# jesselasse/MARL-DMFB

Hardware: AMD Instinct MI355X
Metric: env-steps/sec (whole node), 10x10 DMFB 4-droplet fov9 (higher is better)
Workload: dtype int8 env state/obs + f64 rewards; fp32 Q-net; 1 GPU; DMFB 10x10, drop_num=4, fov=9, 4096 parallel envs per GPU (BASELINE configs[1]); parallelism=dp1: chips sharded per rank, one flat RCCL all-reduce per learn

## Files before the change

marl_dmfb_amd/csrc/gru_ops.hip:

```cpp
#include <hip/hip_runtime.h>

#include <cstdint>
#include <cstdio>
#include <cstdlib>

#include "../../include/crnn_ops.h"

#define HIP_ABI_TAG "crnn_ops"
#define HIP_ABI_ERR CRNN_ERR_HIP
#include "hip_abi.h"

namespace {

constexpr int kBlock = 512;
constexpr int H = 128;
constexpr int RW = 8;
constexpr int KQ = 32;

__device__ __forceinline__ float sigmoidf_(float x) { return 1.0f / (1.0f + __expf(-x)); }

struct SeqOff {
    int32_t packed;
    int32_t off[GRU_SEQ_MAX_STEPS + 1];
};

typedef float f32x2 __attribute__((ext_vector_type(2)));
typedef float f32x4 __attribute__((ext_vector_type(4)));

__global__ __launch_bounds__(kBlock) void k_gru_seq_fwd(const float *__restrict__ igates, const float *__restrict__ h0,
                                                        const float *__restrict__ w_hh, const float *__restrict__ b_ih,
                                                        const float *__restrict__ b_hh, int T, long R,
                                                        float *__restrict__ hs, float *__restrict__ gates, const SeqOff so) {
    __shared__ __attribute__((aligned(16))) float s_h[RW / 2][H][2];
    __shared__ __attribute__((aligned(16))) float s_part[4][RW][3][H];
    const int tid = threadIdx.x, q = tid / H, u = tid - q * H;
    const long row0 = (long)blockIdx.x * RW;
    const int rv = (int)min((long)RW, R - row0);
    f32x4 w[3][KQ / 4];
#pragma unroll
    for (int g = 0; g < 3; ++g)
#pragma unroll
        for (int k = 0; k < KQ / 4; ++k) w[g][k] = *(const f32x4 *)(w_hh + (size_t)(g * H + u) * H + q * KQ + 4 * k);
    const float bir = b_ih[u] + b_hh[u], biz = b_ih[H + u] + b_hh[H + u], bin = b_ih[2 * H + u], bhn = b_hh[2 * H + u];
    for (int i = tid; i < RW * H; i += kBlock) {
        const int rr = i / H, c = i - rr * H;
        s_h[rr >> 1][c][rr & 1] = rr < rv ? h0[(row0 + rr) * H + c] : 0.0f;
    }
    __syncthreads();
    const int ra = 2 * q;
    for (int t = 0; t < T; ++t) {
        const long rt = so.packed ? (long)(so.off[t + 1] - so.off[t]) : R;
        if (row0 >= rt) break;
        const int rvt = (int)min((long)rv, rt - row0);
        const size_t base = so.packed ? (size_t)so.off[t] : (size_t)t * R;
        float ig[2][3];
#pragma unroll
        for (int s = 0; s < 2; ++s) {
            const int rr = ra + s;
#pragma unroll
            for (int g = 0; g < 3; ++g) ig[s][g] = rr < rvt ? igates[(base + row0 + rr) * 3 * H + g * H + u] : 0.0f;
        }
#pragma unroll
        for (int rp = 0; rp < RW / 2; ++rp) {
            const f32x4 *ph = (const f32x4 *)(&s_h[rp][q * KQ][0]);
            f32x2 acc[3] = {{0.0f, 0.0f}, {0.0f, 0.0f}, {0.0f, 0.0f}};
#pragma unroll
            for (int j = 0; j < KQ / 4; ++j) {
                const f32x4 v0 = ph[2 * j], v1 = ph[2 * j + 1];
#pragma unroll
// ... 59 lines not shown
    const int ra = 2 * q;
    float gh[2] = {0.0f, 0.0f};
    float bs_r = 0.0f, bs_z = 0.0f, bs_n = 0.0f, bs_hn = 0.0f;
    int t_last = -1;
    for (int t = 0; t < T; ++t)
        if (row0 < (so.packed ? (long)(so.off[t + 1] - so.off[t]) : R)) t_last = t;
    struct In { float g, rg, zg, ng, hn, hp; };
    In cur[2], nx[2];
    auto fetch = [&](int t, In (&in)[2]) __attribute__((always_inline)) {
        const long rt = so.packed ? (long)(so.off[t + 1] - so.off[t]) : R;
        const int rvt = (int)min((long)rv, rt - row0);
        const size_t base = so.packed ? (size_t)so.off[t] : (size_t)t * R;
        const size_t base_prev = so.packed ? (size_t)so.off[t > 0 ? t - 1 : 0] : (size_t)(t > 0 ? t - 1 : 0) * R;
#pragma unroll
        for (int s = 0; s < 2; ++s) {
            const int rr = ra + s;
            const bool on = rr < rvt;
            const size_t o = base + row0 + (on ? rr : 0);
            in[s].g = on ? grad_hs[o * H + u] : 0.0f;
            in[s].rg = on ? gates[o * 4 * H + u] : 0.0f;
            in[s].zg = on ? gates[o * 4 * H + H + u] : 0.0f;
            in[s].ng = on ? gates[o * 4 * H + 2 * H + u] : 0.0f;
            in[s].hn = on ? gates[o * 4 * H + 3 * H + u] : 0.0f;
            in[s].hp = !on ? 0.0f : t > 0 ? hs[(base_prev + row0 + rr) * H + u] : h0[(row0 + rr) * H + u];
        }
    };
    if (t_last >= 0) fetch(t_last, cur);
    for (int t = t_last; t >= 0; --t) {
        const long rt = so.packed ? (long)(so.off[t + 1] - so.off[t]) : R;
        const int rvt = (int)min((long)rv, rt - row0);
        const size_t base = so.packed ? (size_t)so.off[t] : (size_t)t * R;
        float direct[2];
#pragma unroll
        for (int s = 0; s < 2; ++s) {
            const int rr = ra + s;
            float dpr = 0.0f, dpz = 0.0f, dpn = 0.0f, dhn = 0.0f;
            direct[s] = 0.0f;
            if (rr < rvt) {
                const size_t o = base + row0 + rr;
                const float g = cur[s].g + gh[s];
                const float rg = cur[s].rg, zg = cur[s].zg, ng = cur[s].ng, hn = cur[s].hn;
                const float hp = cur[s].hp;
                if (h_prev_out) h_prev_out[o * H + u] = hp;
                const float dn = g * (1.0f - zg), dz = g * (hp - ng);
                direct[s] = g * zg;
                dpn = dn * (1.0f - ng * ng);
                dhn = dpn * rg;
// ... 136 lines not shown

}

extern "C" {

static int make_seq_off(const int32_t *step_rows, int T, int64_t R, SeqOff &so) {
    so.packed = step_rows ? 1 : 0;
    if (!step_rows) return CRNN_OK;
    if (T > GRU_SEQ_MAX_STEPS) return CRNN_ERR_UNSUPPORTED;
    long off = 0, prev = R;
    for (int t = 0; t < T; ++t) {
        if (step_rows[t] < 0 || step_rows[t] > prev) return CRNN_ERR_BAD_ARG;
        so.off[t] = (int32_t)off;
        off += step_rows[t];
        prev = step_rows[t];
        if (off > 0x7fffffffL) return CRNN_ERR_BAD_ARG;
    }
    so.off[T] = (int32_t)off;
    return CRNN_OK;
}

static int seq_forward(const float *d_igates, const float *d_h0, const float *d_w_hh, const float *d_b_ih, const float *d_b_hh,
                       int T, int64_t R, int hidden, const int32_t *step_rows, float *d_hs, float *d_gates, void *stream) {
    if (!d_igates || !d_h0 || !d_w_hh || !d_b_ih || !d_b_hh || !d_hs || T < 0 || R < 0) return CRNN_ERR_BAD_ARG;
    if (hidden != H) return CRNN_ERR_UNSUPPORTED;
    if (T == 0 || R == 0) return CRNN_OK;
    SeqOff so;
    const int rc = make_seq_off(step_rows, T, R, so);
    if (rc != CRNN_OK) return rc;
    LAUNCH(k_gru_seq_fwd, dim3((unsigned)((R + RW - 1) / RW)), dim3(kBlock), 0, (hipStream_t)stream, d_igates, d_h0, d_w_hh,
           d_b_ih, d_b_hh, T, (long)R, d_hs, d_gates, so);
    return CRNN_OK;
}

int gru_seq_forward(const float *d_igates, const float *d_h0, const float *d_w_hh, const float *d_b_ih, const float *d_b_hh,
                    int T, int64_t R, int hidden, float *d_hs, float *d_gates, void *stream) {
    return seq_forward(d_igates, d_h0, d_w_hh, d_b_ih, d_b_hh, T, R, hidden, nullptr, d_hs, d_gates, stream);
}

int gru_seq_forward_packed(const float *d_igates, const float *d_h0, const float *d_w_hh, const float *d_b_ih, const float *d_b_hh,
                           int T, int64_t R, int hidden, const int32_t *step_rows, float *d_hs, float *d_gates, void *stream) {
    if (!step_rows) return CRNN_ERR_BAD_ARG;
    return seq_forward(d_igates, d_h0, d_w_hh, d_b_ih, d_b_hh, T, R, hidden, step_rows, d_hs, d_gates, stream);
}

int gru_seq_forward_packed_pair(const float *d_igates_a, const float *d_h0_a, const float *d_w_hh_a, const float *d_b_ih_a,
                                const float *d_b_hh_a, float *d_hs_a, float *d_gates_a, const float *d_igates_b, const float *d_h0_b,
                                const float *d_w_hh_b, const float *d_b_ih_b, const float *d_b_hh_b, float *d_hs_b, float *d_gates_b,
                                int T, int64_t R, int hidden, const int32_t *step_rows, void *stream) {
    if (!d_igates_a || !d_w_hh_a || !d_b_ih_a || !d_b_hh_a || !d_hs_a || T < 0 || R < 0 || !step_rows) return CRNN_ERR_BAD_ARG;
    const bool two = d_igates_b != nullptr;
    if (two && (!d_w_hh_b || !d_b_ih_b || !d_b_hh_b || !d_hs_b)) return CRNN_ERR_BAD_ARG;
    if ((((size_t)d_w_hh_a | (size_t)d_w_hh_b) & 15) != 0) return CRNN_ERR_BAD_ARG;
    if (hidden != H) return CRNN_ERR_UNSUPPORTED;
    if (T == 0 || R == 0) return CRNN_OK;
    SeqOff so;
    const int rc = make_seq_off(step_rows, T, R, so);
    if (rc != CRNN_OK) return rc;
    const long per_net = (R + kMW - 1) / kMW;
    if (per_net * 2 > 0x7fffffffL) return CRNN_ERR_BAD_ARG;
    const GruNetIO a{d_igates_a, d_h0_a, d_w_hh_a, d_b_ih_a, d_b_hh_a, d_hs_a, d_gates_a};
    const GruNetIO b{d_igates_b, d_h0_b, d_w_hh_b, d_b_ih_b, d_b_hh_b, d_hs_b, d_gates_b};
    LAUNCH(k_gru_seq_fwd_mfma, dim3((unsigned)(per_net * (two ? 2 : 1))), dim3(kBlock), 0, (hipStream_t)stream, a, two ? b : a,
           (int)per_net, T, (long)R, so);
    return CRNN_OK;
}

static int seq_backward(const float *d_grad_hs, const float *d_gates, const float *d_hs, const float *d_h0, const float *d_w_hh,
                        int T, int64_t R, int hidden, const int32_t *step_rows, float *d_d_igates, float *d_d_hgates, float *d_d_h0,
                        float *d_bias_part, void *stream, float *d_h_prev = nullptr) {
    if (!d_grad_hs || !d_gates || !d_hs || !d_h0 || !d_w_hh || !d_d_igates || !d_d_hgates || T < 0 || R < 0) return CRNN_ERR_BAD_ARG;
    if (hidden != H) return CRNN_ERR_UNSUPPORTED;
    if (T == 0 || R == 0) return CRNN_OK;
    SeqOff so;
    const int rc = make_seq_off(step_rows, T, R, so);
    if (rc != CRNN_OK) return rc;
    LAUNCH(k_gru_seq_bwd, dim3((unsigned)((R + RW - 1) / RW)), dim3(kBlock), 0, (hipStream_t)stream, d_grad_hs, d_gates, d_hs,
           d_h0, d_w_hh, T, (long)R, d_d_igates, d_d_hgates, d_d_h0, d_bias_part, so, d_h_prev);
    return CRNN_OK;
}

int gru_seq_backward(const float *d_grad_hs, const float *d_gates, const float *d_hs, const float *d_h0, const float *d_w_hh,
                     int T, int64_t R, int hidden, float *d_d_igates, float *d_d_hgates, float *d_d_h0, float *d_bias_part,
                     void *stream) {
    return seq_backward(d_grad_hs, d_gates, d_hs, d_h0, d_w_hh, T, R, hidden, nullptr, d_d_igates, d_d_hgates, d_d_h0, d_bias_part, stream);
}

int gru_seq_backward_packed(const float *d_grad_hs, const float *d_gates, const float *d_hs, const float *d_h0, const float *d_w_hh,
                            int T, int64_t R, int hidden, const int32_t *step_rows, float *d_d_igates, float *d_d_hgates,
                            float *d_d_h0, float *d_bias_part, float *d_h_prev, void *stream) {
    if (!step_rows) return CRNN_ERR_BAD_ARG;
    return seq_backward(d_grad_hs, d_gates, d_hs, d_h0, d_w_hh, T, R, hidden, step_rows, d_d_igates, d_d_hgates, d_d_h0, d_bias_part, stream,
                        d_h_prev);
}
// ... 7 lines not shown
```

marl_dmfb_amd/csrc/vdn_ops.hip:

```cpp
#include <hip/hip_runtime.h>

#include <cstdint>

#include "../../include/vdn_ops.h"
#include "../../include/vdn_tail.h"
#include "../../include/vdn_double.h"

#define HIP_ABI_TAG "vdn_ops"
#define HIP_ABI_ERR VDN_ERR_HIP
#include "hip_abi.h"

namespace {

__device__ unsigned g_td_ticket = 0;
__device__ __forceinline__ void td_block_sums(float sq, float mk, float *part, float *__restrict__ sums) {
    __shared__ float s_w[2][4];
    __shared__ int s_last;
    for (int o = 32; o > 0; o >>= 1) { sq += __shfl_xor(sq, o); mk += __shfl_xor(mk, o); }
    if ((threadIdx.x & 63) == 0) { s_w[0][threadIdx.x >> 6] = sq; s_w[1][threadIdx.x >> 6] = mk; }
    __syncthreads();
    if (threadIdx.x < 2) part[2 * blockIdx.x + threadIdx.x] = (s_w[threadIdx.x][0] + s_w[threadIdx.x][1]) + (s_w[threadIdx.x][2] + s_w[threadIdx.x][3]);
    if (!last_workgroup_arrives(&g_td_ticket, gridDim.x, &s_last)) return;
    if (threadIdx.x < 128) {
        const int which = threadIdx.x >> 6;
// ... 129 lines not shown
    }
    const int i = (int)(row % n);
    const UnitOf s = ix.unit(row / n);
    const float d = -((2.0f * mtd[s.row]) * maskf[s.row]) * g[0];
    const int a_taken = (int)u[s.ep * n + i];
    const bool bad_a = (unsigned)a_taken >= (unsigned)A;
    for (int a = 0; a < A; ++a) gq[row * A + a] = (bad_a || a == a_taken) ? d : 0.0f;
}

template <typename V>
__global__ __launch_bounds__(256) void k_gather_units(const V *__restrict__ src, int unit_v, const int32_t *__restrict__ units, int U, int shift,
                                                      int zero_below, V *__restrict__ dst) {
    const long idx = (long)blockIdx.x * blockDim.x + threadIdx.x;
    if (idx >= (long)U * unit_v) return;
    const int j = (int)(idx / unit_v), k = (int)(idx - (long)j * unit_v);
    dst[idx] = j < zero_below ? (V)0 : src[((size_t)units[j] + shift) * unit_v + k];
}

struct GatherBatch {
    const void *src[VDN_GATHER_MAX];
    void *dst[VDN_GATHER_MAX];
    long total[VDN_GATHER_MAX], total_pad[VDN_GATHER_MAX];
    int unit_v[VDN_GATHER_MAX], shift[VDN_GATHER_MAX], zero_below[VDN_GATHER_MAX], dw[VDN_GATHER_MAX];
};
template <typename V>
__device__ __forceinline__ void gather_word(const void *src, int unit_v, const int32_t *__restrict__ units, int shift, int zero_below,
                                            void *dst, long total, long idx) {
    V v = (V)0;
    if (idx < total) {
        const int j = (int)(idx / unit_v), k = (int)(idx - (long)j * unit_v);
        if (j >= zero_below) v = ((const V *)src)[((size_t)units[j] + shift) * unit_v + k];
    }
    ((V *)dst)[idx] = v;
}
__global__ __launch_bounds__(256) void k_gather_units_batch(GatherBatch gb, const int32_t *__restrict__ units) {
    const int d = blockIdx.y;
    const long idx = (long)blockIdx.x * blockDim.x + threadIdx.x;
    if (idx >= gb.total_pad[d]) return;
    if (gb.dw[d]) gather_word<uint32_t>(gb.src[d], gb.unit_v[d], units, gb.shift[d], gb.zero_below[d], gb.dst[d], gb.total[d], idx);
    else gather_word<uint8_t>(gb.src[d], gb.unit_v[d], units, gb.shift[d], gb.zero_below[d], gb.dst[d], gb.total[d], idx);
}

}

#include "vdn_lambda_kernels.h"
#include "vdn_double_kernels.h"

namespace {

struct TensorList {
    float *p[VDN_MAX_TENSORS];
    float *g[VDN_MAX_TENSORS];
    float *m[VDN_MAX_TENSORS];
    float *v[VDN_MAX_TENSORS];
    long off[VDN_MAX_TENSORS + 1];
    int n;
};

__device__ __forceinline__ void locate(const TensorList &tl, long i, int &k) {
    while (i >= tl.off[k + 1]) ++k;
}

__global__ __launch_bounds__(256) void k_sqnorm_partials(TensorList tl, float *__restrict__ partials, const float *__restrict__ grad_div) {
    __shared__ float s_w[4];
    const long total = tl.off[tl.n];
    const long per = (total + gridDim.x - 1) / gridDim.x;
    const long lo = (long)blockIdx.x * per, hi = min(total, lo + per);
    float acc = 0.0f;
    int k = 0;
    for (long i = lo + threadIdx.x; i < hi; i += 256) {
        locate(tl, i, k);
        float g = tl.g[k][i - tl.off[k]];
        if (grad_div) g = g / grad_div[0];
        acc = fmaf(g, g, acc);
    }
    for (int o = 32; o > 0; o >>= 1) acc += __shfl_xor(acc, o);
    if ((threadIdx.x & 63) == 0) s_w[threadIdx.x >> 6] = acc;
    __syncthreads();
    if (threadIdx.x == 0) partials[blockIdx.x] = (s_w[0] + s_w[1]) + (s_w[2] + s_w[3]);
}

__global__ __launch_bounds__(256) void k_clip_adam(TensorList tl, const float *__restrict__ partials, int n_partials, float max_norm,
                                                   float step_size, float omb1, float beta2, float omb2, float eps, float bc2_sqrt,
                                                   float *__restrict__ total_norm, const float *__restrict__ grad_div) {
    __shared__ float s_coef;
    if (threadIdx.x < 64) {
        float t = 0.0f;
        for (int b = threadIdx.x; b < n_partials; b += 64) t += partials[b];
        for (int o = 32; o > 0; o >>= 1) t += __shfl_xor(t, o);
        if (threadIdx.x == 0) {
            const float norm = sqrtf(t);
            s_coef = norm != norm ? norm : fminf(max_norm / (norm + 1e-6f), 1.0f);
            if (blockIdx.x == 0) total_norm[0] = norm;
        }
    }
    __syncthreads();
    const float coef = s_coef;
    const long total = tl.off[tl.n];
    const long per = (total + gridDim.x - 1) / gridDim.x;
    const long lo = (long)blockIdx.x * per, hi = min(total, lo + per);
    int k = 0;
    for (long i = lo + threadIdx.x; i < hi; i += 256) {
        locate(tl, i, k);
        const long j = i - tl.off[k];
        float g = tl.g[k][j];
        if (grad_div) g = g / grad_div[0];
        g = g * coef;
        if (grad_div || coef != 1.0f) tl.g[k][j] = g;
        float m = tl.m[k][j], v = tl.v[k][j];
        m = m + omb1 * (g - m);
        v = beta2 * v + omb2 * g * g;
        tl.m[k][j] = m;
        tl.v[k][j] = v;
        const float denom = sqrtf(v) / bc2_sqrt + eps;
        tl.p[k][j] -= step_size * (m / denom);
    }
}

bool td_forward_args_ok(const TdIn &in, const TdOut &out) {
    return !(out.sums && !out.part) && in.qe && in.qt && in.u && in.r && in.avail && in.term && in.padded && out.mtd && out.maskf && in.n >= 1 &&
           in.A >= 1 && in.A <= 127;
}
bool td_backward_args_ok(const float *mtd, const float *mask, const int8_t *u, const float *g, const float *gq, int n, int A) {
    return mtd && mask && u && g && gq && n >= 1 && A >= 1 && A <= 127;
}
bool padded_shape_ok(int B, int T, int Tl) { return B >= 0 && T >= 1 && Tl >= T; }

int td_no_rows(const TdOut &out, void *stream) {
    if (out.sums) HIP_TRY(hipMemsetAsync(out.sums, 0, 2 * sizeof(float), (hipStream_t)stream));
    return VDN_OK;
}

bool lambda_padded_args_ok(const TdIn &in, const TdOut &out, int B, int T, int Tl, float lam) {
    return td_forward_args_ok(in, out) && padded_shape_ok(B, T, Tl) && T <= VDN_LAMBDA_MAX_T && lam >= 0.0f && lam <= 1.0f &&
           (int64_t)B * T <= 0x7fffffffL;
}
bool lambda_packed_args_ok(const TdIn &in, const TdOut &out, const int32_t *units, int n_units, float lam, int n_steps) {
    return td_forward_args_ok(in, out) && units && n_units >= 0 && lam >= 0.0f && lam <= 1.0f && n_steps >= 0 && n_steps <= VDN_LAMBDA_MAX_T;
// ... 224 lines not shown
    return VDN_OK;
}

int vdn_gather_units_batch(int32_t n_gathers, const void *const *d_src, const int32_t *unit_bytes, const int32_t *unit_shift,
                           const int32_t *zero_below, void *const *d_dst, const int64_t *dst_bytes, const int32_t *d_units,
                           int32_t n_units, void *stream) {
    if (n_gathers < 1 || n_gathers > VDN_GATHER_MAX || !d_src || !unit_bytes || !unit_shift || !zero_below || !d_dst || !dst_bytes ||
        !d_units || n_units < 0)
        return VDN_ERR_BAD_ARG;
    GatherBatch gb{};
    long most = 0;
    for (int i = 0; i < n_gathers; ++i) {
        if (!d_src[i] || !d_dst[i] || unit_bytes[i] < 1 || zero_below[i] < 0 || dst_bytes[i] < (int64_t)n_units * unit_bytes[i])
            return VDN_ERR_BAD_ARG;
        const bool dw = unit_bytes[i] % 4 == 0 && dst_bytes[i] % 4 == 0 && ((size_t)d_src[i] | (size_t)d_dst[i]) % 4 == 0;
        gb.src[i] = d_src[i];
        gb.dst[i] = d_dst[i];
        gb.dw[i] = dw ? 1 : 0;
        gb.unit_v[i] = dw ? unit_bytes[i] / 4 : unit_bytes[i];
        gb.total[i] = (long)n_units * gb.unit_v[i];
        gb.total_pad[i] = (long)(dw ? dst_bytes[i] / 4 : dst_bytes[i]);
        gb.shift[i] = unit_shift[i];
        gb.zero_below[i] = zero_below[i];
        most = gb.total_pad[i] > most ? gb.total_pad[i] : most;
    }
    if (most == 0) return VDN_OK;
    if ((most + 255) / 256 > 0x7fffffffL) return VDN_ERR_BAD_ARG;
    LAUNCH(k_gather_units_batch, dim3((unsigned)((most + 255) / 256), (unsigned)n_gathers), dim3(256), 0, (hipStream_t)stream, gb, d_units);
    return VDN_OK;
}

int vdn_last_hip_error(void) { return g_last_hip; }

}
```

marl_dmfb_amd/network/base_net.py:

```python

import torch
import torch.nn as nn
import torch.nn.functional as f


_CONV_PLAN = {5: [(True, 1)], 7: [(True, 1), (False, 1)], 9: [(True, 1), (False, 1)], 11: [(True, 1), (False, 1)],
              13: [(True, 1), (False, 1)], 19: [(True, 2), (False, 1), (False, 1)]}


class _ConvGemm(torch.autograd.Function):

    @staticmethod
    def forward(ctx, cols, weight2d, bias):
        ctx.save_for_backward(cols, weight2d)
        return torch.addmm(bias, cols, weight2d.t())

    @staticmethod
    def backward(ctx, g):
        cols, w = ctx.saved_tensors
        g = g.contiguous()
        gcols = g @ w if ctx.needs_input_grad[0] else None
        M, K = cols.shape
        C = g.shape[1]
        S = 1
# ... 344 lines not shown
        h0c, w = h0.contiguous(), w_hh.contiguous()
        d_ig = torch.empty((T, R, 3 * H), dtype=torch.float32, device=hs.device)
        d_hg = torch.empty_like(d_ig)
        d_h0 = torch.empty_like(h0c)
        bias_part = torch.empty((lib.gru_seq_row_blocks(R), 6 * H), dtype=torch.float32, device=hs.device)
        lib.gru_seq_backward(grad_out.data_ptr(), gates.data_ptr(), hs.data_ptr(), h0c.data_ptr(),
                             w.data_ptr(), T, R, H, d_ig.data_ptr(), d_hg.data_ptr(), d_h0.data_ptr(),
                             bias_part.data_ptr(), torch.cuda.current_stream(hs.device).cuda_stream)
        d_w_hh = torch.matmul(d_hg[0].t(), h0c)
        if T > 1:
            d_w_hh = d_w_hh + _wgrad_splitk(d_hg[1:].reshape((T - 1) * R, 3 * H), hs[:-1].reshape((T - 1) * R, H))
        d_b = bias_part.sum(0)
        return d_ig, d_h0, d_w_hh, d_b[:3 * H], d_b[3 * H:]


class _GRUSeqHipPacked(torch.autograd.Function):

    @staticmethod
    def _steps(step_rows):
        import ctypes as C
        return (C.c_int32 * len(step_rows))(*[int(v) for v in step_rows])

    @staticmethod
    def run_forward(igates, h0, w_hh, b_ih, b_hh, step_rows, save):
        lib = _GRUSeqHip._lib()
        Vp, G = igates.shape
        H, T, R, V = G // 3, len(step_rows), h0.shape[0], int(sum(step_rows))
        igates, h0, w_hh = igates.contiguous(), h0.contiguous(), w_hh.contiguous()
        hs = torch.empty((Vp, H), dtype=torch.float32, device=igates.device)
        hs[V:].zero_()
        gates = torch.empty((Vp, 4 * H), dtype=torch.float32, device=igates.device) if save else None
        lib.gru_seq_forward_packed(igates.data_ptr(), h0.data_ptr(), w_hh.data_ptr(), b_ih.data_ptr(),
                                   b_hh.data_ptr(), T, R, H, _GRUSeqHipPacked._steps(step_rows), hs.data_ptr(),
                                   gates.data_ptr() if save else None,
                                   torch.cuda.current_stream(igates.device).cuda_stream)
        return hs, gates

    @staticmethod
    def forward(ctx, igates, h0, w_hh, b_ih, b_hh, step_rows):
        hs, gates = _GRUSeqHipPacked.run_forward(igates.detach(), h0.detach(), w_hh.detach(), b_ih.detach(), b_hh.detach(), step_rows, True)
        ctx.save_for_backward(hs, gates, h0, w_hh)
        ctx.step_rows = list(step_rows)
        return hs

    @staticmethod
    def backward(ctx, grad_out):
        hs, gates, h0, w_hh = ctx.saved_tensors
        lib = _GRUSeqHip._lib()
        step_rows = ctx.step_rows
        Vp, H = hs.shape
        T, R, V = len(step_rows), h0.shape[0], int(sum(step_rows))
        grad_out = grad_out.contiguous()
        h0c, w = h0.contiguous(), w_hh.contiguous()
        d_ig = torch.empty((Vp, 3 * H), dtype=torch.float32, device=hs.device)
        d_hg = torch.empty_like(d_ig)
        h_prev = torch.empty((Vp, H), dtype=torch.float32, device=hs.device)
        for t in (d_ig, d_hg, h_prev):
            t[V:].zero_()
        d_h0 = torch.zeros_like(h0c)
        bias_part = torch.empty((lib.gru_seq_row_blocks(R), 6 * H), dtype=torch.float32, device=hs.device)
        lib.gru_seq_backward_packed(grad_out.data_ptr(), gates.data_ptr(), hs.data_ptr(), h0c.data_ptr(),
                                    w.data_ptr(), T, R, H, _GRUSeqHipPacked._steps(step_rows), d_ig.data_ptr(),
                                    d_hg.data_ptr(), d_h0.data_ptr(), bias_part.data_ptr(), h_prev.data_ptr(),
                                    torch.cuda.current_stream(hs.device).cuda_stream)
        d_w_hh = _wgrad_splitk(d_hg, h_prev)
        d_b = bias_part.sum(0)
        return d_ig, d_h0, d_w_hh, d_b[:3 * H], d_b[3 * H:], None


class _GRUSeqPairPacked(torch.autograd.Function):

    @staticmethod
    def forward(ctx, ig_a, w_hh_a, b_ih_a, b_hh_a, ig_b, w_hh_b, b_ih_b, b_hh_b, step_rows, R):
        lib = _GRUSeqHip._lib()
        Vp, G = ig_a.shape
        Hd, T, V = G // 3, len(step_rows), int(sum(step_rows))
        save = any(ctx.needs_input_grad[:4])
        ta = [t.detach().contiguous() for t in (ig_a, w_hh_a, b_ih_a, b_hh_a)]
        tb = [t.detach().contiguous() for t in (ig_b, w_hh_b, b_ih_b, b_hh_b)]
        hs_a = torch.empty((Vp, Hd), dtype=torch.float32, device=ig_a.device)
        hs_b = torch.empty((Vp, Hd), dtype=torch.float32, device=ig_a.device)
        hs_a[V:].zero_()
        hs_b[V:].zero_()
        gates = torch.empty((Vp, 4 * Hd), dtype=torch.float32, device=ig_a.device) if save else None
        lib.gru_seq_forward_packed_pair(ta[0].data_ptr(), None, ta[1].data_ptr(), ta[2].data_ptr(), ta[3].data_ptr(),
                                        hs_a.data_ptr(), gates.data_ptr() if save else None,
                                        tb[0].data_ptr(), None, tb[1].data_ptr(), tb[2].data_ptr(), tb[3].data_ptr(),
                                        hs_b.data_ptr(), None, T, R, Hd, _GRUSeqHipPacked._steps(step_rows),
                                        torch.cuda.current_stream(ig_a.device).cuda_stream)
        if save:
            h0 = torch.zeros((R, Hd), dtype=torch.float32, device=ig_a.device)
            ctx.save_for_backward(hs_a, gates, h0, ta[1])
            ctx.step_rows = list(step_rows)
        ctx.mark_non_differentiable(hs_b)
        return hs_a, hs_b

    @staticmethod
    def backward(ctx, grad_a, _grad_b):
        d_ig, _d_h0, d_w_hh, d_b_ih, d_b_hh, _ = _GRUSeqHipPacked.backward(ctx, grad_a)
        return d_ig, d_w_hh, d_b_ih, d_b_hh, None, None, None, None, None, None


def gru_sequence(igates, h0, w_hh, b_ih, b_hh, impl='hip'):
    if impl == 'hip' and h0.shape[-1] == 128 and igates.dtype == torch.float32:
        if torch.is_grad_enabled() and any(t.requires_grad for t in (igates, h0, w_hh, b_ih, b_hh)):
            return _GRUSeqHip.apply(igates, h0, w_hh, b_ih, b_hh)
        return _GRUSeqHip.run_forward(igates, h0, w_hh, b_ih, b_hh, False)[0]
    return _GRUSeq.apply(igates, h0, w_hh, b_ih, b_hh)


def conv_str(fov, id=3, od=32):
    stack, shared = [], None
    for from_image, stride in _CONV_PLAN[fov]:
        if from_image:
            stack.append(nn.Conv2d(id, od, kernel_size=3, stride=stride))
        else:
            if shared is None:
                shared = nn.Conv2d(od, od, kernel_size=3, stride=stride)
            stack.append(shared)
    return stack


# ... 49 lines not shown
        return self.fc1(h), h

    def recurrent_seq(self, x_seq, h0):
        T, R = x_seq.shape[0], x_seq.shape[1]
        h = h0.reshape(-1, self.rnn_hidden_dim)
        hs = []
        if x_seq.is_cuda:
            w_ih = self.weight_ih_padded() if x_seq.shape[-1] == self.padded_cols() != self.rnn.weight_ih.shape[1] else self.rnn.weight_ih
            igates = _LinearSplitK.apply(x_seq.reshape(T * R, -1), w_ih, None).view(T, R, -1)
            hseq = gru_sequence(igates, h, self.rnn.weight_hh, self.rnn.bias_ih, self.rnn.bias_hh,
                                getattr(self, 'gru_impl', 'hip'))
            q = _LinearSplitK.apply(hseq.view(T * R, -1), self.fc1.weight, self.fc1.bias).view(T, R, -1)
            return q, hseq[-1]
        else:
            for t in range(T):
                h = self.rnn(x_seq[t], h)
                hs.append(h)
        q = self.fc1(torch.stack(hs, dim=0).view(T * R, -1)).view(T, R, -1)
        return q, h

    def recurrent_seq_packed(self, x, step_rows, R, return_hidden=False):
        w_ih = self.weight_ih_padded() if x.shape[-1] == self.padded_cols() != self.rnn.weight_ih.shape[1] else self.rnn.weight_ih
        igates = _LinearSplitK.apply(x, w_ih, None)
        h0 = torch.zeros((R, self.rnn_hidden_dim), dtype=torch.float32, device=x.device)
        args = (igates, h0, self.rnn.weight_hh, self.rnn.bias_ih, self.rnn.bias_hh)
        if torch.is_grad_enabled() and any(t.requires_grad for t in args):
            hs = _GRUSeqHipPacked.apply(*args, step_rows)
        else:
            hs = _GRUSeqHipPacked.run_forward(*args, step_rows, False)[0]
        q = _LinearSplitK.apply(hs, self.fc1.weight, self.fc1.bias)
        return (q, hs.detach()) if return_hidden else q

    @staticmethod
    def recurrent_seq_packed_pair(net_a, x_a, net_b, x_b, step_rows, R, return_hidden=False):
        def w_ih(net, x, grad):
            if x.shape[-1] == net.padded_cols() != net.rnn.weight_ih.shape[1]:
                return net.weight_ih_padded() if grad else net.refresh_padded()
            return net.rnn.weight_ih
        ig_a = _LinearSplitK.apply(x_a, w_ih(net_a, x_a, True), None)
        with torch.no_grad():
            ig_b = torch.matmul(x_b, w_ih(net_b, x_b, False).t())
        hs_a, hs_b = _GRUSeqPairPacked.apply(ig_a, net_a.rnn.weight_hh, net_a.rnn.bias_ih, net_a.rnn.bias_hh,
                                             ig_b, net_b.rnn.weight_hh.detach(), net_b.rnn.bias_ih.detach(), net_b.rnn.bias_hh.detach(),
                                             step_rows, R)
        q_a = _LinearSplitK.apply(hs_a, net_a.fc1.weight, net_a.fc1.bias)
        with torch.no_grad():
            q_b = torch.addmm(net_b.fc1.bias, hs_b, net_b.fc1.weight.t())
        return (q_a, q_b, hs_a.detach()) if return_hidden else (q_a, q_b)

    def forward(self, inputs, hidden_state):
        return self.recurrent(self.features(inputs), hidden_state)

# ... 174 lines not shown
```

marl_dmfb_amd/policy/vdn.py:

```python
import os

import torch

from ..network.base_net import CRNN, RNN
from ..network.vdn_net import VDNNet


def _t(x, device, dtype):
    if not isinstance(x, torch.Tensor):
        x = torch.as_tensor(x)
    return x.to(device=device, dtype=dtype)


def _episode_slots(t):
    inner = 1
    for k in range(t.dim() - 1, 0, -1):
        if t.stride(k) != inner and t.shape[k] != 1:
            return None
        inner *= t.shape[k]
    per_step = inner // t.shape[1]
    if t.shape[0] == 1:
        return t.shape[1]
    if per_step == 0 or t.stride(0) % per_step or t.stride(0) // per_step < t.shape[1]:
        return None
# ... 1 lines not shown


def _td_forward(ctx, form, head, rows, episodes, dev, bad, lam, lam_tail=(), sel=None):
    from .. import _lib
    lib = _lib.checked('vdn_lambda' if lam else 'vdn_tail')
    mtd = torch.empty(rows, dtype=torch.float32, device=dev)
    mask = torch.empty(rows, dtype=torch.float32, device=dev)
    sums = torch.empty(2, dtype=torch.float32, device=dev)
    part = torch.empty(lib.vdn_td_lambda_sum_parts(episodes) if lam else lib.vdn_td_sum_parts(rows), dtype=torch.float32, device=dev)
    out = (mtd.data_ptr(), mask.data_ptr(), None if bad is None else bad.data_ptr(), part.data_ptr(), sums.data_ptr())
    stream = torch.cuda.current_stream(dev).cuda_stream
    if sel is None:
        entry = getattr(lib, 'vdn_td_%sforward%s_sums' % ('lambda_' if lam else '', form))
        entry(*head, *out, *((float(lam), None) + tuple(lam_tail) if lam else ()), stream)
    else:
        sel_args, n, picks_out = sel
        picks = None if picks_out is None else torch.empty((rows, n), dtype=torch.int8, device=dev)
        entry = getattr(_lib.checked('vdn_double'), 'vdn_td_double_forward%s_sums' % form)
        entry(*head, *out, float(lam), None, *lam_tail, *sel_args, None if picks is None else picks.data_ptr(), stream)
        if picks is not None:
            picks_out.append(picks)
    num, mask_sum = sums[0], sums[1]
    ctx.mark_non_differentiable(mask_sum)
    return mtd, mask, num, mask_sum


class _TDLoss(torch.autograd.Function):

    @staticmethod
    def forward(ctx, q_eval_tm, q_target_tm, u, r, avail_next, terminated, padded, T, gamma, bad=None, lam=0.0, q_sel=None, picks=None):
        B, n, A = u.shape[0], u.shape[2], avail_next.shape[3]
        t_limit = _episode_slots(u)
        q_eval_tm, q_target_tm = q_eval_tm.contiguous(), q_target_tm.contiguous()
        head = [t.data_ptr() for t in (q_eval_tm, q_target_tm, u, r, avail_next, terminated, padded)]
        sel = None
        if q_sel is not None:
            q_sel = q_sel.contiguous()
            sel = ((q_sel.data_ptr(),), n, picks)
        mtd, mask, num, mask_sum = _td_forward(ctx, '', head + [B, T, t_limit, n, A, float(gamma)], B * T, B, u.device, bad, lam, (), sel)
        ctx.save_for_backward(mtd, mask, u)
        ctx.dims = (B, T, t_limit, n, A)
        return num, mask_sum

    @staticmethod
    def backward(ctx, g_num, _g_mask):
        from .. import _lib
        lib = _lib.checked('vdn_ops')
        mtd, mask, u = ctx.saved_tensors
        B, T, t_limit, n, A = ctx.dims
        gq = torch.empty((T, B * n, A), dtype=torch.float32, device=u.device)
        g = g_num.reshape(1).to(torch.float32).contiguous()
        lib.vdn_td_backward(mtd.data_ptr(), mask.data_ptr(), u.data_ptr(), g.data_ptr(), B, T, t_limit, n, A,
                            gq.data_ptr(), torch.cuda.current_stream(u.device).cuda_stream)
        return (gq,) + (None,) * 12


class _TDLossPacked(torch.autograd.Function):

    @staticmethod
    def forward(ctx, q_eval, q_target, units, n_units, u, r, avail_next, terminated, padded, n, A, gamma, bad=None, lam=0.0,
                counts=None, q_sel=None, sel_units=None, picks=None):
        import ctypes as C
        steps = [int(c) for c in counts] if lam else []
        q_eval, q_target = q_eval.contiguous(), q_target.contiguous()
        head = [q_eval.data_ptr(), q_target.data_ptr(), units.data_ptr(), n_units] + \
               [t.data_ptr() for t in (u, r, avail_next, terminated, padded)] + [n, A, float(gamma)]
        sel = None
        if q_sel is not None:
            q_sel = q_sel.contiguous()
            sel = ((q_sel.data_ptr(), q_sel.shape[0] // n, None if sel_units is None else sel_units.data_ptr()), n, picks)
        mtd, mask, num, mask_sum = _td_forward(ctx, '_packed', head, n_units, steps[0] if steps else 0, u.device, bad, lam,
                                               (len(steps), (C.c_int32 * len(steps))(*steps) if steps else None), sel)
        ctx.save_for_backward(mtd, mask, units, u)
        ctx.dims = (n_units, n, A, q_eval.shape[0])
        return num, mask_sum

    @staticmethod
    def backward(ctx, g_num, _g_mask):
        from .. import _lib
        lib = _lib.checked('vdn_tail')
        mtd, mask, units, u = ctx.saved_tensors
        n_units, n, A, rows_pad = ctx.dims
        gq = torch.empty((rows_pad, A), dtype=torch.float32, device=u.device)
        g = g_num.reshape(1).to(torch.float32).contiguous()
        lib.vdn_td_backward_packed_pad(mtd.data_ptr(), mask.data_ptr(), units.data_ptr(), n_units, u.data_ptr(),
                                       g.data_ptr(), n, A, rows_pad, gq.data_ptr(), torch.cuda.current_stream(u.device).cuda_stream)
        return (gq,) + (None,) * 17


PACK_ROWS = 2048


class VDN:
    def __init__(self, args):
        self.args = args
        self.n_actions = args.n_actions
        self.n_agents = args.n_agents
        input_shape = args.obs_shape[-1]
        if args.last_action:
            input_shape += self.n_actions
        if args.reuse_network:
            input_shape += self.n_agents
        if args.net == 'rnn':
# ... 193 lines not shown

        self.optimizer.zero_grad()
        if self.dist:
            num = (masked_td_error ** 2).sum()
            num.backward()
            total = self._allreduce_grads(mask.sum())
            return self._step_and_sync(num.detach() / total, train_step, grad_div=total)
        loss = (masked_td_error ** 2).sum() / mask.sum()
        loss.backward()
        return self._step_and_sync(loss, train_step)

    def _td_lambda(self):
        lam = getattr(self.args, 'td_lambda', 0.0)
        if not lam:
            return 0.0
        from .td_lambda import check_lambda
        return check_lambda(lam)

    def _double_q(self):
        return bool(getattr(self.args, 'double_q', False))

    def _backward_and_step(self, num, mask_sum, train_step):
        self.optimizer.zero_grad()
        num.backward()
        total = self._allreduce_grads(mask_sum) if self.dist else mask_sum
        return self._step_and_sync(num.detach() / total, train_step, grad_div=total)

    def packed_ok(self, buffers):
        return bool(self.args.alg == 'vdn' and len(list(self.eval_vdn_net.parameters())) == 0 and self._packed_front_ok(buffers))

    def _packed_front_ok(self, buffers):
        net = self.eval_rnn
        o = buffers.get('o')
        if not (isinstance(o, torch.Tensor) and o.is_cuda and o.dtype == torch.int8 and o.is_contiguous()
                and self.args.last_action and hasattr(net, 'recurrent_seq_packed') and getattr(net, 'rnn_hidden_dim', 0) == 128
                and o.shape[1] <= 255):
            return False
        want = {'u': torch.int8, 'r': torch.float32, 'avail_u_next': torch.int8, 'terminated': torch.bool, 'padded': torch.bool,
                'u_onehot': torch.int8, 'o_next': torch.int8}
        if any(not (isinstance(buffers.get(k), torch.Tensor) and buffers[k].dtype == dt and buffers[k].is_contiguous()) for k, dt in want.items()):
            return False
        probe = o.view(-1, o.shape[-1])[:1]
        with torch.no_grad():
            return bool(hasattr(net, '_hip_conv_ok') and net._hip_conv_ok(probe) and hasattr(net, '_hip_train_ok')
                        and net._hip_front() in (5, 7, 9, 11, 13, 19))

    @staticmethod
    def pack_units(idx, lens, t_ring):
        import numpy as np
# ... 260 lines not shown
```

Baseline: 7.815 million env-steps/s.

## Drop zero h0 allocations, vectorize unit gather, prefetch Adam and norm loops

Several independent changes. The GRU forward and backward kernels now accept a null h0 and treat it as zeros, so the packed path no longer allocates and reads zero-filled initial hidden states or their gradients. The unit gather kernel processes four elements per thread, with vectorized stores and 32-bit index math when sizes allow. The squared-norm and Adam kernels keep four elements in flight per thread, and Adam prefetches its first batch while the partial sums are being reduced. On the Python side, a cached ones tensor seeds backward and autograd grad materialization is disabled, which cuts small per-step allocations and launches at the cost of extra code paths and None handling.

New measurement: 7.903 million env-steps/s (median of 6 runs). +1.1%, better.

```diff
diff --git a/marl_dmfb_amd/csrc/gru_ops.hip b/marl_dmfb_amd/csrc/gru_ops.hip
--- a/marl_dmfb_amd/csrc/gru_ops.hip
+++ b/marl_dmfb_amd/csrc/gru_ops.hip
@@ -44,7 +44,7 @@
     const float bir = b_ih[u] + b_hh[u], biz = b_ih[H + u] + b_hh[H + u], bin = b_ih[2 * H + u], bhn = b_hh[2 * H + u];
     for (int i = tid; i < RW * H; i += kBlock) {
         const int rr = i / H, c = i - rr * H;
-        s_h[rr >> 1][c][rr & 1] = rr < rv ? h0[(row0 + rr) * H + c] : 0.0f;
+        s_h[rr >> 1][c][rr & 1] = (rr < rv && h0) ? h0[(row0 + rr) * H + c] : 0.0f;
     }
     __syncthreads();
     const int ra = 2 * q;
@@ -150,7 +150,7 @@
             in[s].zg = on ? gates[o * 4 * H + H + u] : 0.0f;
             in[s].ng = on ? gates[o * 4 * H + 2 * H + u] : 0.0f;
             in[s].hn = on ? gates[o * 4 * H + 3 * H + u] : 0.0f;
-            in[s].hp = !on ? 0.0f : t > 0 ? hs[(base_prev + row0 + rr) * H + u] : h0[(row0 + rr) * H + u];
+            in[s].hp = !on ? 0.0f : t > 0 ? hs[(base_prev + row0 + rr) * H + u] : h0 ? h0[(row0 + rr) * H + u] : 0.0f;
         }
     };
     if (t_last >= 0) fetch(t_last, cur);
@@ -333,7 +333,7 @@
 
 static int seq_forward(const float *d_igates, const float *d_h0, const float *d_w_hh, const float *d_b_ih, const float *d_b_hh,
                        int T, int64_t R, int hidden, const int32_t *step_rows, float *d_hs, float *d_gates, void *stream) {
-    if (!d_igates || !d_h0 || !d_w_hh || !d_b_ih || !d_b_hh || !d_hs || T < 0 || R < 0) return CRNN_ERR_BAD_ARG;
+    if (!d_igates || !d_w_hh || !d_b_ih || !d_b_hh || !d_hs || T < 0 || R < 0) return CRNN_ERR_BAD_ARG;
     if (hidden != H) return CRNN_ERR_UNSUPPORTED;
     if (T == 0 || R == 0) return CRNN_OK;
     SeqOff so;
@@ -380,7 +380,7 @@
 static int seq_backward(const float *d_grad_hs, const float *d_gates, const float *d_hs, const float *d_h0, const float *d_w_hh,
                         int T, int64_t R, int hidden, const int32_t *step_rows, float *d_d_igates, float *d_d_hgates, float *d_d_h0,
                         float *d_bias_part, void *stream, float *d_h_prev = nullptr) {
-    if (!d_grad_hs || !d_gates || !d_hs || !d_h0 || !d_w_hh || !d_d_igates || !d_d_hgates || T < 0 || R < 0) return CRNN_ERR_BAD_ARG;
+    if (!d_grad_hs || !d_gates || !d_hs || !d_w_hh || !d_d_igates || !d_d_hgates || T < 0 || R < 0) return CRNN_ERR_BAD_ARG;
     if (hidden != H) return CRNN_ERR_UNSUPPORTED;
     if (T == 0 || R == 0) return CRNN_OK;
     SeqOff so;
diff --git a/marl_dmfb_amd/csrc/vdn_ops.hip b/marl_dmfb_amd/csrc/vdn_ops.hip
--- a/marl_dmfb_amd/csrc/vdn_ops.hip
+++ b/marl_dmfb_amd/csrc/vdn_ops.hip
@@ -175,23 +175,57 @@
     void *dst[VDN_GATHER_MAX];
     long total[VDN_GATHER_MAX], total_pad[VDN_GATHER_MAX];
     int unit_v[VDN_GATHER_MAX], shift[VDN_GATHER_MAX], zero_below[VDN_GATHER_MAX], dw[VDN_GATHER_MAX];
-};
-template <typename V>
-__device__ __forceinline__ void gather_word(const void *src, int unit_v, const int32_t *__restrict__ units, int shift, int zero_below,
-                                            void *dst, long total, long idx) {
-    V v = (V)0;
-    if (idx < total) {
-        const int j = (int)(idx / unit_v), k = (int)(idx - (long)j * unit_v);
-        if (j >= zero_below) v = ((const V *)src)[((size_t)units[j] + shift) * unit_v + k];
-    }
-    ((V *)dst)[idx] = v;
+    int vec[VDN_GATHER_MAX];
+    int narrow;
+};
+template <typename V> struct Four;
+template <> struct Four<uint32_t> { typedef uint4 type; };
+template <> struct Four<uint8_t> { typedef uchar4 type; };
+template <typename V, typename I>
+__device__ __forceinline__ void gather_four(const void *src, int unit_v, const int32_t *__restrict__ units, int shift, int zero_below,
+                                            void *dst, bool vec, I total, I total_pad, I idx0) {
+    V v[4] = {(V)0, (V)0, (V)0, (V)0};
+    if (idx0 < total) {
+        I j = idx0 / (I)unit_v, k = idx0 - j * (I)unit_v;
+        bool on[4];
+        I kk[4];
+        int un[4];
+#pragma unroll
+        for (int w = 0; w < 4; ++w) {
+            on[w] = idx0 + (I)w < total && (long)j >= (long)zero_below;
+            kk[w] = k;
+            un[w] = units[on[w] ? j : (I)0];
+            if (++k == (I)unit_v) { k = 0; ++j; }
+        }
+#pragma unroll
+        for (int w = 0; w < 4; ++w) {
+            const V x = ((const V *)src)[on[w] ? ((size_t)un[w] + shift) * unit_v + kk[w] : (size_t)0];
+            v[w] = on[w] ? x : (V)0;
+        }
+    }
+    if (vec && idx0 + (I)3 < total_pad) {
+        typename Four<V>::type o;
+        o.x = v[0]; o.y = v[1]; o.z = v[2]; o.w = v[3];
+        *(typename Four<V>::type *)((V *)dst + idx0) = o;
+    } else {
+#pragma unroll
+        for (int w = 0; w < 4; ++w)
+            if (idx0 + (I)w < total_pad) ((V *)dst)[idx0 + (I)w] = v[w];
+    }
 }
 __global__ __launch_bounds__(256) void k_gather_units_batch(GatherBatch gb, const int32_t *__restrict__ units) {
     const int d = blockIdx.y;
-    const long idx = (long)blockIdx.x * blockDim.x + threadIdx.x;
-    if (idx >= gb.total_pad[d]) return;
-    if (gb.dw[d]) gather_word<uint32_t>(gb.src[d], gb.unit_v[d], units, gb.shift[d], gb.zero_below[d], gb.dst[d], gb.total[d], idx);
-    else gather_word<uint8_t>(gb.src[d], gb.unit_v[d], units, gb.shift[d], gb.zero_below[d], gb.dst[d], gb.total[d], idx);
+    const long idx0 = 4 * ((long)blockIdx.x * blockDim.x + threadIdx.x);
+    if (idx0 >= gb.total_pad[d]) return;
+    const bool vec = gb.vec[d] != 0;
+    if (gb.narrow) {
+        const uint32_t t = (uint32_t)gb.total[d], tp = (uint32_t)gb.total_pad[d], i0 = (uint32_t)idx0;
+        if (gb.dw[d]) gather_four<uint32_t, uint32_t>(gb.src[d], gb.unit_v[d], units, gb.shift[d], gb.zero_below[d], gb.dst[d], vec, t, tp, i0);
+        else gather_four<uint8_t, uint32_t>(gb.src[d], gb.unit_v[d], units, gb.shift[d], gb.zero_below[d], gb.dst[d], vec, t, tp, i0);
+    } else {
+        if (gb.dw[d]) gather_four<uint32_t, long>(gb.src[d], gb.unit_v[d], units, gb.shift[d], gb.zero_below[d], gb.dst[d], vec, gb.total[d], gb.total_pad[d], idx0);
+        else gather_four<uint8_t, long>(gb.src[d], gb.unit_v[d], units, gb.shift[d], gb.zero_below[d], gb.dst[d], vec, gb.total[d], gb.total_pad[d], idx0);
+    }
 }
 
 }
@@ -213,19 +247,34 @@
 __device__ __forceinline__ void locate(const TensorList &tl, long i, int &k) {
     while (i >= tl.off[k + 1]) ++k;
 }
+constexpr int kFly = 4;
 
 __global__ __launch_bounds__(256) void k_sqnorm_partials(TensorList tl, float *__restrict__ partials, const float *__restrict__ grad_div) {
     __shared__ float s_w[4];
     const long total = tl.off[tl.n];
     const long per = (total + gridDim.x - 1) / gridDim.x;
     const long lo = (long)blockIdx.x * per, hi = min(total, lo + per);
+    const bool div = grad_div != nullptr;
+    const float gd = div ? grad_div[0] : 1.0f;
     float acc = 0.0f;
     int k = 0;
-    for (long i = lo + threadIdx.x; i < hi; i += 256) {
-        locate(tl, i, k);
-        float g = tl.g[k][i - tl.off[k]];
-        if (grad_div) g = g / grad_div[0];
-        acc = fmaf(g, g, acc);
+    for (long i = lo + threadIdx.x; i < hi; i += 256 * kFly) {
+        float g[kFly];
+#pragma unroll
+        for (int s = 0; s < kFly; ++s) {
+            const long e = i + 256 * s;
+            g[s] = 0.0f;
+            if (e < hi) {
+                locate(tl, e, k);
+                g[s] = tl.g[k][e - tl.off[k]];
+            }
+        }
+#pragma unroll
+        for (int s = 0; s < kFly; ++s)
+            if (i + 256 * s < hi) {
+                const float x = div ? g[s] / gd : g[s];
+                acc = fmaf(x, x, acc);
+            }
     }
     for (int o = 32; o > 0; o >>= 1) acc += __shfl_xor(acc, o);
     if ((threadIdx.x & 63) == 0) s_w[threadIdx.x >> 6] = acc;
@@ -237,9 +286,38 @@
                                                    float step_size, float omb1, float beta2, float omb2, float eps, float bc2_sqrt,
                                                    float *__restrict__ total_norm, const float *__restrict__ grad_div) {
     __shared__ float s_coef;
-    if (threadIdx.x < 64) {
+    const int tid = threadIdx.x;
+    const long total = tl.off[tl.n];
+    const long per = (total + gridDim.x - 1) / gridDim.x;
+    const long lo = (long)blockIdx.x * per, hi = min(total, lo + per);
+    const bool div = grad_div != nullptr;
+    float x0 = 0.0f, x1 = 0.0f;
+    if (tid < 64) {
+        if (tid < n_partials) x0 = partials[tid];
+        if (tid + 64 < n_partials) x1 = partials[tid + 64];
+    }
+    const float gd = div ? grad_div[0] : 1.0f;
+    struct El { float *g, *m, *v, *p; float gv, mv, vv, pv; };
+    El el[kFly];
+    int k = 0;
+    auto fetch = [&](long i) __attribute__((always_inline)) {
+#pragma unroll
+        for (int s = 0; s < kFly; ++s) {
+            const long e = i + 256 * s;
+            if (e < hi) {
+                locate(tl, e, k);
+                const long j = e - tl.off[k];
+                el[s].g = tl.g[k] + j; el[s].m = tl.m[k] + j; el[s].v = tl.v[k] + j; el[s].p = tl.p[k] + j;
+                el[s].gv = *el[s].g; el[s].mv = *el[s].m; el[s].vv = *el[s].v; el[s].pv = *el[s].p;
+            }
+        }
+    };
+    fetch(lo + tid);
+    if (tid < 64) {
         float t = 0.0f;
-        for (int b = threadIdx.x; b < n_partials; b += 64) t += partials[b];
+        if (tid < n_partials) t += x0;
+        if (tid + 64 < n_partials) t += x1;
+        for (int b = tid + 128; b < n_partials; b += 64) t += partials[b];
         for (int o = 32; o > 0; o >>= 1) t += __shfl_xor(t, o);
         if (threadIdx.x == 0) {
             const float norm = sqrtf(t);
@@ -249,24 +327,23 @@
     }
     __syncthreads();
     const float coef = s_coef;
-    const long total = tl.off[tl.n];
-    const long per = (total + gridDim.x - 1) / gridDim.x;
-    const long lo = (long)blockIdx.x * per, hi = min(total, lo + per);
-    int k = 0;
-    for (long i = lo + threadIdx.x; i < hi; i += 256) {
-        locate(tl, i, k);
-        const long j = i - tl.off[k];
-        float g = tl.g[k][j];
-        if (grad_div) g = g / grad_div[0];
-        g = g * coef;
-        if (grad_div || coef != 1.0f) tl.g[k][j] = g;
-        float m = tl.m[k][j], v = tl.v[k][j];
-        m = m + omb1 * (g - m);
-        v = beta2 * v + omb2 * g * g;
-        tl.m[k][j] = m;
-        tl.v[k][j] = v;
-        const float denom = sqrtf(v) / bc2_sqrt + eps;
-        tl.p[k][j] -= step_size * (m / denom);
+    for (long i = lo + tid; i < hi; i += 256 * kFly) {
+        if (i != lo + tid) fetch(i);
+#pragma unroll
+        for (int s = 0; s < kFly; ++s) {
+            if (i + 256 * s >= hi) continue;
+            float g = el[s].gv;
+            if (div) g = g / gd;
+            g = g * coef;
+            if (div || coef != 1.0f) *el[s].g = g;
+            float m = el[s].mv, v = el[s].vv;
+            m = m + omb1 * (g - m);
+            v = beta2 * v + omb2 * g * g;
+            *el[s].m = m;
+            *el[s].v = v;
+            const float denom = sqrtf(v) / bc2_sqrt + eps;
+            *el[s].p = el[s].pv - step_size * (m / denom);
+        }
     }
 }
 
@@ -537,11 +614,14 @@
         gb.total_pad[i] = (long)(dw ? dst_bytes[i] / 4 : dst_bytes[i]);
         gb.shift[i] = unit_shift[i];
         gb.zero_below[i] = zero_below[i];
+        gb.vec[i] = (size_t)d_dst[i] % (dw ? 16 : 4) == 0 ? 1 : 0;
         most = gb.total_pad[i] > most ? gb.total_pad[i] : most;
     }
     if (most == 0) return VDN_OK;
-    if ((most + 255) / 256 > 0x7fffffffL) return VDN_ERR_BAD_ARG;
-    LAUNCH(k_gather_units_batch, dim3((unsigned)((most + 255) / 256), (unsigned)n_gathers), dim3(256), 0, (hipStream_t)stream, gb, d_units);
+    gb.narrow = most + 4 <= 0x7fffffffL ? 1 : 0;
+    const long threads = (most + 3) / 4;
+    if ((threads + 255) / 256 > 0x7fffffffL) return VDN_ERR_BAD_ARG;
+    LAUNCH(k_gather_units_batch, dim3((unsigned)((threads + 255) / 256), (unsigned)n_gathers), dim3(256), 0, (hipStream_t)stream, gb, d_units);
     return VDN_OK;
 }
 
diff --git a/marl_dmfb_amd/network/base_net.py b/marl_dmfb_amd/network/base_net.py
--- a/marl_dmfb_amd/network/base_net.py
+++ b/marl_dmfb_amd/network/base_net.py
@@ -390,25 +390,28 @@
         return (C.c_int32 * len(step_rows))(*[int(v) for v in step_rows])
 
     @staticmethod
-    def run_forward(igates, h0, w_hh, b_ih, b_hh, step_rows, save):
+    def run_forward(igates, h0, w_hh, b_ih, b_hh, step_rows, save, R=None):
         lib = _GRUSeqHip._lib()
         Vp, G = igates.shape
-        H, T, R, V = G // 3, len(step_rows), h0.shape[0], int(sum(step_rows))
-        igates, h0, w_hh = igates.contiguous(), h0.contiguous(), w_hh.contiguous()
+        H, T, R, V = G // 3, len(step_rows), int(R) if h0 is None else h0.shape[0], int(sum(step_rows))
+        igates, w_hh = igates.contiguous(), w_hh.contiguous()
+        h0 = None if h0 is None else h0.contiguous()
         hs = torch.empty((Vp, H), dtype=torch.float32, device=igates.device)
         hs[V:].zero_()
         gates = torch.empty((Vp, 4 * H), dtype=torch.float32, device=igates.device) if save else None
-        lib.gru_seq_forward_packed(igates.data_ptr(), h0.data_ptr(), w_hh.data_ptr(), b_ih.data_ptr(),
+        lib.gru_seq_forward_packed(igates.data_ptr(), None if h0 is None else h0.data_ptr(), w_hh.data_ptr(), b_ih.data_ptr(),
                                    b_hh.data_ptr(), T, R, H, _GRUSeqHipPacked._steps(step_rows), hs.data_ptr(),
                                    gates.data_ptr() if save else None,
                                    torch.cuda.current_stream(igates.device).cuda_stream)
         return hs, gates
 
     @staticmethod
-    def forward(ctx, igates, h0, w_hh, b_ih, b_hh, step_rows):
-        hs, gates = _GRUSeqHipPacked.run_forward(igates.detach(), h0.detach(), w_hh.detach(), b_ih.detach(), b_hh.detach(), step_rows, True)
+    def forward(ctx, igates, h0, w_hh, b_ih, b_hh, step_rows, R=None):
+        hs, gates = _GRUSeqHipPacked.run_forward(igates.detach(), None if h0 is None else h0.detach(), w_hh.detach(), b_ih.detach(),
+                                                 b_hh.detach(), step_rows, True, R)
         ctx.save_for_backward(hs, gates, h0, w_hh)
         ctx.step_rows = list(step_rows)
+        ctx.R = int(R) if h0 is None else h0.shape[0]
         return hs
 
     @staticmethod
@@ -417,23 +420,23 @@
         lib = _GRUSeqHip._lib()
         step_rows = ctx.step_rows
         Vp, H = hs.shape
-        T, R, V = len(step_rows), h0.shape[0], int(sum(step_rows))
+        T, R, V = len(step_rows), ctx.R, int(sum(step_rows))
         grad_out = grad_out.contiguous()
-        h0c, w = h0.contiguous(), w_hh.contiguous()
+        h0c, w = None if h0 is None else h0.contiguous(), w_hh.contiguous()
         d_ig = torch.empty((Vp, 3 * H), dtype=torch.float32, device=hs.device)
         d_hg = torch.empty_like(d_ig)
         h_prev = torch.empty((Vp, H), dtype=torch.float32, device=hs.device)
         for t in (d_ig, d_hg, h_prev):
             t[V:].zero_()
-        d_h0 = torch.zeros_like(h0c)
+        d_h0 = None if h0c is None else torch.zeros_like(h0c)
         bias_part = torch.empty((lib.gru_seq_row_blocks(R), 6 * H), dtype=torch.float32, device=hs.device)
-        lib.gru_seq_backward_packed(grad_out.data_ptr(), gates.data_ptr(), hs.data_ptr(), h0c.data_ptr(),
+        lib.gru_seq_backward_packed(grad_out.data_ptr(), gates.data_ptr(), hs.data_ptr(), None if h0c is None else h0c.data_ptr(),
                                     w.data_ptr(), T, R, H, _GRUSeqHipPacked._steps(step_rows), d_ig.data_ptr(),
-                                    d_hg.data_ptr(), d_h0.data_ptr(), bias_part.data_ptr(), h_prev.data_ptr(),
+                                    d_hg.data_ptr(), None if d_h0 is None else d_h0.data_ptr(), bias_part.data_ptr(), h_prev.data_ptr(),
                                     torch.cuda.current_stream(hs.device).cuda_stream)
         d_w_hh = _wgrad_splitk(d_hg, h_prev)
         d_b = bias_part.sum(0)
-        return d_ig, d_h0, d_w_hh, d_b[:3 * H], d_b[3 * H:], None
+        return d_ig, d_h0, d_w_hh, d_b[:3 * H], d_b[3 * H:], None, None
 
 
 class _GRUSeqPairPacked(torch.autograd.Function):
@@ -457,15 +460,18 @@
                                         hs_b.data_ptr(), None, T, R, Hd, _GRUSeqHipPacked._steps(step_rows),
                                         torch.cuda.current_stream(ig_a.device).cuda_stream)
         if save:
-            h0 = torch.zeros((R, Hd), dtype=torch.float32, device=ig_a.device)
-            ctx.save_for_backward(hs_a, gates, h0, ta[1])
+            ctx.save_for_backward(hs_a, gates, None, ta[1])
             ctx.step_rows = list(step_rows)
+            ctx.R = int(R)
         ctx.mark_non_differentiable(hs_b)
+        ctx.set_materialize_grads(False)
         return hs_a, hs_b
 
     @staticmethod
     def backward(ctx, grad_a, _grad_b):
-        d_ig, _d_h0, d_w_hh, d_b_ih, d_b_hh, _ = _GRUSeqHipPacked.backward(ctx, grad_a)
+        if grad_a is None:
+            return (None,) * 10
+        d_ig, _d_h0, d_w_hh, d_b_ih, d_b_hh, _, _ = _GRUSeqHipPacked.backward(ctx, grad_a)
         return d_ig, d_w_hh, d_b_ih, d_b_hh, None, None, None, None, None, None
 
 
@@ -561,12 +567,11 @@
     def recurrent_seq_packed(self, x, step_rows, R, return_hidden=False):
         w_ih = self.weight_ih_padded() if x.shape[-1] == self.padded_cols() != self.rnn.weight_ih.shape[1] else self.rnn.weight_ih
         igates = _LinearSplitK.apply(x, w_ih, None)
-        h0 = torch.zeros((R, self.rnn_hidden_dim), dtype=torch.float32, device=x.device)
-        args = (igates, h0, self.rnn.weight_hh, self.rnn.bias_ih, self.rnn.bias_hh)
-        if torch.is_grad_enabled() and any(t.requires_grad for t in args):
-            hs = _GRUSeqHipPacked.apply(*args, step_rows)
+        args = (igates, None, self.rnn.weight_hh, self.rnn.bias_ih, self.rnn.bias_hh)
+        if torch.is_grad_enabled() and any(t.requires_grad for t in args if t is not None):
+            hs = _GRUSeqHipPacked.apply(*args, step_rows, R)
         else:
-            hs = _GRUSeqHipPacked.run_forward(*args, step_rows, False)[0]
+            hs = _GRUSeqHipPacked.run_forward(*args, step_rows, False, R)[0]
         q = _LinearSplitK.apply(hs, self.fc1.weight, self.fc1.bias)
         return (q, hs.detach()) if return_hidden else q
 
diff --git a/marl_dmfb_amd/policy/vdn.py b/marl_dmfb_amd/policy/vdn.py
--- a/marl_dmfb_amd/policy/vdn.py
+++ b/marl_dmfb_amd/policy/vdn.py
@@ -47,6 +47,7 @@
             picks_out.append(picks)
     num, mask_sum = sums[0], sums[1]
     ctx.mark_non_differentiable(mask_sum)
+    ctx.set_materialize_grads(False)
     return mtd, mask, num, mask_sum
 
 
@@ -71,6 +72,8 @@
     def backward(ctx, g_num, _g_mask):
         from .. import _lib
         lib = _lib.checked('vdn_ops')
+        if g_num is None:
+            return (None,) * 13
         mtd, mask, u = ctx.saved_tensors
         B, T, t_limit, n, A = ctx.dims
         gq = torch.empty((T, B * n, A), dtype=torch.float32, device=u.device)
@@ -104,6 +107,8 @@
     def backward(ctx, g_num, _g_mask):
         from .. import _lib
         lib = _lib.checked('vdn_tail')
+        if g_num is None:
+            return (None,) * 18
         mtd, mask, units, u = ctx.saved_tensors
         n_units, n, A, rows_pad = ctx.dims
         gq = torch.empty((rows_pad, A), dtype=torch.float32, device=u.device)
@@ -343,9 +348,15 @@
 
     def _backward_and_step(self, num, mask_sum, train_step):
         self.optimizer.zero_grad()
-        num.backward()
+        num.backward(self._grad_one(num))
         total = self._allreduce_grads(mask_sum) if self.dist else mask_sum
         return self._step_and_sync(num.detach() / total, train_step, grad_div=total)
+
+    def _grad_one(self, num):
+        one = getattr(self, '_one', None)
+        if one is None or one.device != num.device or one.dtype != num.dtype or one.shape != num.shape:
+            one = self._one = torch.ones_like(num)
+        return one
 
     def packed_ok(self, buffers):
         return bool(self.args.alg == 'vdn' and len(list(self.eval_vdn_net.parameters())) == 0 and self._packed_front_ok(buffers))
```
